# baggepinnen/LPVSpectral.jl

Measured on AMD Instinct MI355X. Metric: signals/sec, ls_sparse_spectral_lpv group lasso N=2^20 Nf=512 Nv=8 (2000 ADMM iters; iters/sec in admm_iters_per_sec), higher is better.
Workload: dtype f64

## Files before the change

lpvspectral.jl_amd/csrc/admm_pack.hip:

```cpp
#include "lpvs_internal.h"
#include "admm_device.h"
#include "admm_host.h"

#include <algorithm>
#include <map>
#include <mutex>
#include <tuple>
#include <vector>
#include <cmath>
#include <cstdlib>
#include <string>
#include <type_traits>

namespace lpvs {

namespace {

__global__ void __launch_bounds__(256)
pack_tiles_f32_kernel(const double *__restrict__ M, int64_t np, float *__restrict__ Mp) {
    int I, J;
    tile_index(blockIdx.x, I, J);
    const double2 *src = reinterpret_cast<const double2 *>(M + (int64_t)I * TS * np + (int64_t)J * TS);
    float2 *dst = reinterpret_cast<float2 *>(Mp + (int64_t)blockIdx.x * TS * TS);
    for (int e = threadIdx.x; e < TS * TS / 2; e += 256) {
// ... 27 lines not shown
}

__global__ void __launch_bounds__(256)
pack_tiles_split_kernel(const double *__restrict__ M, int64_t np, unsigned char *__restrict__ Mp) {
    int I, J;
    tile_index(blockIdx.x, I, J);
    M += (int64_t)blockIdx.y * np * np;
    Mp += (size_t)blockIdx.y * gridDim.x * kSplitTileBytes;
    const double *src = M + (int64_t)I * TS * np + (int64_t)J * TS;
    float *head = reinterpret_cast<float *>(Mp + (size_t)blockIdx.x * kSplitTileBytes);
    unsigned short *tail = reinterpret_cast<unsigned short *>(Mp + (size_t)blockIdx.x * kSplitTileBytes + (size_t)TS * TS * 4);
    for (int e = threadIdx.x; e < TS * TS; e += 256) {
        const int r = e >> 7, col = e & 127;
        const double m = src[(int64_t)r * np + col];
        unsigned long long B = (unsigned long long)__double_as_longlong(m);
        B = (B + (1ull << 12)) & ~((1ull << 13) - 1);
        float h = (float)__longlong_as_double((long long)(B & ~((1ull << 29) - 1)));
        unsigned int q = (unsigned int)(B >> 13) & 0xffffu;
        if (!(fabs(m) >= 0x1p-120) || !(fabs(m) < 0x1p127)) { h = (float)m; q = 0; }
        head[e] = h;
        tail[r * TS + 8 * ((col & 63) >> 2) + 4 * (col >> 6) + (col & 3)] = (unsigned short)q;
    }
}

__global__ void __launch_bounds__(256)
absmax_kernel(const double *__restrict__ M, int64_t np, int64_t n, unsigned long long *__restrict__ out) {
    M += (int64_t)blockIdx.y * np * np;
    out += blockIdx.y;
    double m = 0.0;
    for (int64_t i = (int64_t)blockIdx.x * 256 + threadIdx.x; i < n; i += (int64_t)gridDim.x * 256) m = fmax(m, fabs(M[i * np + i]));
#pragma unroll
    for (int w = 32; w >= 1; w >>= 1) m = fmax(m, __shfl_xor(m, w, 64));
    if ((threadIdx.x & 63) == 0 && m > 0.0) atomicMax(out, (unsigned long long)__double_as_longlong(m));
}

__global__ void __launch_bounds__(256)
pack_tiles_mixed_kernel(const double *__restrict__ M, int64_t np, unsigned char *__restrict__ Mp, unsigned char *__restrict__ types,
                        const unsigned long long *__restrict__ absmax_bits, double step_scale, int diag_float ,
                        double *__restrict__ abs1 , double *__restrict__ abs2 ,
                        int fix_drop_bits ) {
    int I, J;
    tile_index(blockIdx.x, I, J);
    M += (int64_t)blockIdx.y * np * np;
    Mp += (size_t)blockIdx.y * gridDim.x * kSplitTileBytes;
    types += (size_t)blockIdx.y * gridDim.x;
    absmax_bits += blockIdx.y;
    const double *src = M + (int64_t)I * TS * np + (int64_t)J * TS;
    unsigned char *slot = Mp + (size_t)blockIdx.x * kSplitTileBytes;
    __shared__ float rowstep[TS];
    __shared__ int bad;
    __shared__ double colabs[4][TS];
    const int lane = threadIdx.x & 63, wave = threadIdx.x >> 6;
    if (threadIdx.x == 0) bad = (diag_float && I == J) ? 1 : 0;
    __syncthreads();
    {
        const double limit = __longlong_as_double((long long)*absmax_bits) * step_scale;
        double c0 = 0.0, c1 = 0.0;
        for (int r = wave; r < TS; r += 4) {
            const double a0 = fabs(src[(int64_t)r * np + lane]), a1 = fabs(src[(int64_t)r * np + 64 + lane]);
            if (abs1 != nullptr) {
                c0 += a0; c1 += a1;
                const double rs = wave_sum(a0 + a1);
                if (lane == 0) abs1[(size_t)blockIdx.x * TS + r] = rs;
            }
            const double e0 = (I == J && lane == r) ? 0.0 : a0;
            const double e1 = (I == J && 64 + lane == r) ? 0.0 : a1;
            double m = fmax(e0, e1);
#pragma unroll
            for (int w = 32; w >= 1; w >>= 1) m = fmax(m, __shfl_xor(m, w, 64));
            if (lane == 0) {
                int e = 0;
                (void)frexp(m, &e);
                const double st = ldexp(1.0, e - 35);
                rowstep[r] = m > 0.0 ? (float)st : 0x1p-100f;
                if (m > 0.0 && (!(st <= limit) || e - 35 < -120)) atomicOr(&bad, 1);
            }
        }
        if (abs1 != nullptr) { colabs[wave][lane] = c0; colabs[wave][64 + lane] = c1; }
    }
    __syncthreads();
    if (abs2 != nullptr && threadIdx.x < TS)
        abs2[(size_t)blockIdx.x * TS + threadIdx.x] = ((colabs[0][threadIdx.x] + colabs[1][threadIdx.x]) + colabs[2][threadIdx.x]) + colabs[3][threadIdx.x];
    const bool fixed = !bad;
    if (threadIdx.x == 0) types[blockIdx.x] = fixed ? (I == J ? 2 : 1) : 0;
    if (!fixed) {
        float *head = reinterpret_cast<float *>(slot);
        unsigned short *tail = reinterpret_cast<unsigned short *>(slot + (size_t)TS * TS * 4);
        for (int e = threadIdx.x; e < TS * TS; e += 256) {
            const int r = e >> 7, col = e & 127;
            const double m = src[(int64_t)r * np + col];
            unsigned long long B = (unsigned long long)__double_as_longlong(m);
            B = (B + (1ull << 12)) & ~((1ull << 13) - 1);
            float h = (float)__longlong_as_double((long long)(B & ~((1ull << 29) - 1)));
            unsigned int q = (unsigned int)(B >> 13) & 0xffffu;
            if (!(fabs(m) >= 0x1p-120) || !(fabs(m) < 0x1p127)) { h = (float)m; q = 0; }
            head[e] = h;
            tail[r * TS + 8 * ((col & 63) >> 2) + 4 * (col >> 6) + (col & 3)] = (unsigned short)q;
        }
        return;
    }
    const double drop = (double)(1 << fix_drop_bits), drop_inv = 1.0 / drop;
    unsigned int *hi = reinterpret_cast<unsigned int *>(slot);
    unsigned int *nib = reinterpret_cast<unsigned int *>(slot + kFixHeadBytes);
    float *steps = reinterpret_cast<float *>(slot + kFixHeadBytes + kFixNibBytes);
    const int g = lane >> 4, c = lane & 15;
    for (int rg = 0; rg < 8; ++rg) {
        const int r = wave * 32 + 4 * rg + g;
        const double inv = 1.0 / (double)rowstep[r];
        unsigned int word = 0;
#pragma unroll
        for (int k = 0; k < 8; ++k) {
            const int col = k < 4 ? 4 * c + k : 64 + 4 * c + (k - 4);
            double qd = (I == J && col == r) ? 0.0 : rint(src[(int64_t)r * np + col] * inv * drop_inv) * drop;
            qd = fmin(fmax(qd, -0x1p35 + 1.0), 0x1p35 - 1.0);
            const unsigned long long q = (unsigned long long)((long long)qd + (1ll << 35));
            hi[r * TS + col] = (unsigned int)(q >> 4);
            word |= (unsigned int)(q & 15) << (4 * k);
        }
        nib[(wave * 64 + lane) * 8 + rg] = word;
        if (c == 0) steps[(wave * 4 + g) * 8 + rg] = rowstep[r];
    }
    if (I == J && threadIdx.x < TS)
        reinterpret_cast<double *>(slot + kFixHeadBytes + kFixNibBytes + TS * 4)[threadIdx.x] = src[(int64_t)threadIdx.x * np + threadIdx.x];
}

}

int32_t launch_pack_tiles_batch(const double *M, int64_t np, int nbatch, double *Mp, hipStream_t s) {
    const int nblk = (int)(np / TS);
    hipLaunchKernelGGL(pack_tiles_kernel, dim3((unsigned)(nblk * (nblk + 1) / 2), (unsigned)nbatch), dim3(256), 0, s, M, np, Mp);
    LPVS_HIP(hipGetLastError());
    return LPVS_OK;
}

size_t symv_part_doubles(int64_t np, int64_t ns) {
    const int64_t nblk = np / TS;
    return ((size_t)(nblk * (nblk + 1) / 2) * TS * 2 + 2 * (size_t)nblk + 2) * (size_t)ns + 16;
}
size_t symv_packed_doubles(int64_t np) {
    const int64_t nblk = np / TS;
    return (size_t)(nblk * (nblk + 1) / 2) * TS * TS;
}

int32_t launch_pack_tiles_f32(const double *M, int64_t np, float *Mp, hipStream_t s) {
    const int nblk = (int)(np / TS);
    hipLaunchKernelGGL(pack_tiles_f32_kernel, dim3((unsigned)(nblk * (nblk + 1) / 2)), dim3(256), 0, s, M, np, Mp);
    LPVS_HIP(hipGetLastError());
    return LPVS_OK;
}

int32_t launch_cvt_f32_f64(const float *src, double *dst, int64_t count, hipStream_t s) {
    if (count <= 0) return LPVS_OK;
    hipLaunchKernelGGL(cvt_f32_f64_kernel, dim3((unsigned)ceil_div(count, 256)), dim3(256), 0, s, src, dst, count);
// ... 67 lines not shown
```

lpvspectral.jl_amd/csrc/api.hip:

```cpp
#include <cmath>
#include <cstdarg>
#include <cstdio>
#include <cstdlib>
#include <cstring>
#include <ctime>
#include <map>
#include <mutex>
#include <array>
#include <thread>
#include <string>
#include <vector>

#include "lpvs_internal.h"

namespace lpvs {

static thread_local char g_err[512] = "";

void set_error(const char *fmt, ...) {
    va_list ap;
    va_start(ap, fmt);
    vsnprintf(g_err, sizeof(g_err), fmt, ap);
    va_end(ap);
}
// ... 448 lines not shown

AdmmParams make_params(const lpvs_problem *h) {
    const StoragePlan &pl = h->plan;
    const bool sym = h->np >= kSymmetricMinNp;
    AdmmParams p{h->M.as<double>(), h->np, h->n, h->bs.as<double>(), h->x.as<double>(), h->z.as<double>(), h->u.as<double>(),
                 h->rhs.as<double>(), h->mu, h->tol, h->prox_kind, h->prox_param, h->group_len, h->status.as<AdmmStatus>(),
                 h->scratch.as<double>(), h->part.as<double>(), sym ? h->Mp.as<double>() : nullptr, (int)h->ns};
    p.mp_f32 = pl.mode == kMpF32 ? 1 : 0;
    p.mp_split = pl.mode == kMpSplit || pl.mode == kMpMixed ? 1 : 0;
    p.mp_types = pl.mode == kMpMixed ? mp_tile_types(h->Mp, h->np, 1) : nullptr;
    p.mp_fix32 = p.mp_types != nullptr && (pl.fix_bits <= 32 || pl.nib_period > 0) ? 1 : 0;
    p.nib_period = pl.nib_period; p.nib_ramp = pl.nib_ramp; p.xb_corr = h->xb_corr.as<double>(); p.nib_rhs = h->nib_rhs.as<double>(); p.nib_part = h->nib_part.as<double>(); p.nib_acc = h->nib_acc.as<long long>();
    p.xb = pl.offset_form ? h->xb.as<double>() : nullptr;
    p.fi = pl.owns_fi && h->fi.p ? h->fi.as<double>() : nullptr;
    p.fi_R = h->fi_R; p.fi_xbmax = h->fi_xbmax;
    p.fi_prefetch_all = pl.mode == kMpMixed && h->Mp_census.fixed == h->Mp_census.total ? 1 : 0;
    p.opt_iteration = h->opt[LPVS_OPT_ITERATION]; p.opt_nt_loads = h->opt[LPVS_OPT_NT_LOADS];
    {
        const char *e = experiment_env("LPVS_TILE_ORDER");
        p.tile_order = p.fi != nullptr && !(e && std::string(e) == "forward") ? 1 : 0;
    }
    p.sm_ctl = !sym && h->sm_ctl.p ? h->sm_ctl.as<int>() : nullptr;
    p.prox_params = h->prox_per_signal && h->ns > 1 ? h->prox_params.as<double>() : nullptr;
    return p;
}

int32_t factorize(lpvs_problem *h, double shift) {
    if (h->M_valid && h->M_shift == shift) return LPVS_OK;
    const int64_t np = h->np, n = h->n;
    h->Mp_valid = false; h->Mp_rowsum = 0;
    if (!h->M.p) LPVS_TRY(h->M.alloc(sizeof(double) * (size_t)np * (size_t)np));
    if (!h->work.p) LPVS_TRY(h->work.alloc(spd_inverse_work_bytes(np)));
    LPVS_HIP(hipEventRecord(h->ev[3].a, h->stream));
    LPVS_HIP(hipMemcpyAsync(h->M.p, h->G.p, sizeof(double) * (size_t)np * (size_t)np, hipMemcpyDeviceToDevice, h->stream));
    LPVS_TRY(launch_add_diag(h->M.as<double>(), np, n, shift, h->stream));
    LPVS_TRY(spd_inverse_inplace(h->M.as<double>(), np, h->work.as<double>(), h->istat.as<int>(), h->stream, &h->res->aux));
    LPVS_HIP(hipEventRecord(h->ev[3].b, h->stream));
    int st = 0;
    LPVS_HIP(hipMemcpyAsync(&st, h->istat.p, sizeof(int), hipMemcpyDeviceToHost, h->stream));
    LPVS_HIP(hipStreamSynchronize(h->stream));
    h->t_factor += h->ev[3].ms();
    if (st != 0) {
        h->M_valid = false;
        set_error("(G + %.3g I) is not positive definite (non-positive pivot in the block sweep)", shift);
        return LPVS_ENUMERIC;
    }
    h->M_valid = true; h->M_shift = shift;
    return LPVS_OK;
}


StoragePlan decide_plan(lpvs_problem *h) {
    const int xc_opt = option_in_effect(LPVS_OPT_XUPDATE_CORRECTION, h->opt[LPVS_OPT_XUPDATE_CORRECTION]);
    const bool corrected = h->np >= kSymmetricMinNp && xc_opt != LPVS_XCORR_OFF;
    h->xcorr = xcorr_schedule_from(corrected ? experiment_env("LPVS_XUPDATE_CORRECTION") : nullptr, xcorr_default_schedule(h->ns, corrected));
    const int storage = option_in_effect(LPVS_OPT_M_STORAGE, h->opt[LPVS_OPT_M_STORAGE]);
    return admm_storage_plan(h->np, h->ns, h->f32, storage, h->ns > 1 && multi_signal_fixed_tiles_ok(h->np), h->xcorr.on(), fix_bits_from(experiment_env),
                             nib_knobs_from(experiment_env));
}

int32_t pack_mixed(lpvs_problem *h, const StoragePlan &want, StoragePlan *stored) {
    hipStream_t s = h->stream;
    const PackedLayout lay = packed_layout(h->np, want.element_bytes, 1);
    unsigned char *types = mp_tile_types(h->Mp, h->np, 1);
    unsigned long long *amax = reinterpret_cast<unsigned long long *>(h->Mp.as<unsigned char>() + lay.absmax_off);
    LPVS_TRY(launch_pack_tiles_mixed(h->M.as<double>(), h->np, h->Mp.as<unsigned char>(), types, amax, s, want.diag_float,
                                     want.want_rowsum ? h->part.as<double>() : nullptr, h->n, want.want_rowsum ? h->scratch.as<double>() : nullptr, want.fix_bits));
    std::vector<unsigned char> ht(lay.tiles);
// ... 2134 lines not shown
```

lpvspectral.jl_amd/csrc/linalg.hip:

```cpp
#include "lpvs_internal.h"
#include "factor_plan.h"

#include <cstdlib>
#include <map>
#include <mutex>
#include <string>
#include <vector>

namespace lpvs {

namespace {

typedef double f64x4 __attribute__((ext_vector_type(4)));
constexpr int NB = 64;

__global__ void __launch_bounds__(256)
diag_inverse_kernel(const double *__restrict__ Aall, int64_t np, int k, double *__restrict__ Pall, int *status,
                    int64_t strideA, int64_t strideW) {
    __shared__ double colp[NB], rowp[NB];
    const double *A = Aall + (int64_t)blockIdx.x * strideA;
    double *P = Pall + (int64_t)blockIdx.x * strideW;
    const double *blk = A + (int64_t)k * NB * np + (int64_t)k * NB;
    const int ti = threadIdx.x >> 4, tj = threadIdx.x & 15;
    double v[4][4];
// ... 864 lines not shown
            }
        }
        __syncthreads();
    }
    if (skip_wave) return;
    if (below) {
#pragma unroll
        for (int i = 0; i < 2; ++i)
#pragma unroll
            for (int r = 0; r < 4; ++r) {
                double *sp = A + (r_lo + i * 16 + 4 * r) * np + c_lo;
#pragma unroll
                for (int j = 0; j < 2; ++j) *reinterpret_cast<double *>(reinterpret_cast<char *>(sp + j * 16) + voffb) = acc[i][j][r];
            }
        return;
    }
#pragma unroll
    for (int i = 0; i < 2; ++i)
#pragma unroll
        for (int j = 0; j < 2; ++j)
#pragma unroll
            for (int r = 0; r < 4; ++r) {
                const int64_t row = r_lo + i * 16 + lk + 4 * r, col = c_lo + j * 16 + li;
                if (col <= row) A[row * np + col] = acc[i][j][r];
            }
}

__global__ void __launch_bounds__(256) add_diag_kernel(double *__restrict__ Mall, int64_t np, int64_t n, double shift) {
    const int64_t i = (int64_t)blockIdx.x * 256 + threadIdx.x;
    double *M = Mall + (int64_t)blockIdx.y * np * np;
    if (i < np) M[i * np + i] = i < n ? M[i * np + i] + shift : 1.0;
}

__global__ void __launch_bounds__(256) negate_mirror_kernel(double *__restrict__ Aall, int64_t np) {
    __shared__ double tile[32][33];
    double *A = Aall + (int64_t)blockIdx.z * np * np;
    const int bi = blockIdx.y, bj = blockIdx.x;
    if (bj > bi) return;
    const int tx = threadIdx.x & 31, ty = threadIdx.x >> 5;
    const int64_t r0 = (int64_t)bi * 32, c0 = (int64_t)bj * 32;
    for (int r = ty; r < 32; r += 8) {
        const double v = -A[(r0 + r) * np + c0 + tx];
        tile[r][tx] = v;
        if (bi != bj || tx <= r) A[(r0 + r) * np + c0 + tx] = v;
    }
    __syncthreads();
    for (int r = ty; r < 32; r += 8)
        if (bi != bj || tx > r) A[(c0 + r) * np + r0 + tx] = tile[tx][r];
}

__global__ void __launch_bounds__(256)
symm_matmul_kernel(const double *__restrict__ A, const double *__restrict__ B, double *__restrict__ C, int64_t np) {
    const int lane = threadIdx.x & 63, wave = threadIdx.x >> 6;
    const int64_t r0 = ((int64_t)blockIdx.y * 2 + (wave >> 1)) * 64, c0 = ((int64_t)blockIdx.x * 2 + (wave & 1)) * 64;
    const int li = lane & 15, lk = lane >> 4;
    f64x4 acc[4][4];
#pragma unroll
    for (int i = 0; i < 4; ++i)
#pragma unroll
        for (int j = 0; j < 4; ++j) acc[i][j] = (f64x4){0.0, 0.0, 0.0, 0.0};
    for (int64_t kk = 0; kk < np; kk += 4) {
        double opA[4], opB[4];
#pragma unroll
        for (int q = 0; q < 4; ++q) {
            opA[q] = A[(kk + lk) * np + r0 + q * 16 + li];
            opB[q] = B[(kk + lk) * np + c0 + q * 16 + li];
// ... 325 lines not shown
    }
    return factor_steps_serial(c, plan);
}

static int32_t spd_inverse_impl(double *A, int64_t np, int nbatch, double *work, int *status_dev, hipStream_t s, SweepAux *aux) {
    if (np % 128 != 0) { set_error("spd_inverse: np=%lld not a multiple of 128", (long long)np); return LPVS_ESTATE; }
    LPVS_HIP(hipMemsetAsync(status_dev, 0, sizeof(int) * (size_t)nbatch, s));
    const FactorPlan plan = factor_plan(np, nbatch, aux != nullptr, factor_knobs_from(experiment_env));
    if (plan.level == FactorLevel::two) {
        LPVS_TRY(spd_inverse_two_level(A, np, work, status_dev, s, aux, plan));
    } else {
        sweep64(A, np, nbatch, work, status_dev, s);
        LPVS_HIP(hipGetLastError());
    }
    hipLaunchKernelGGL(negate_mirror_kernel, dim3((unsigned)(np / 32), (unsigned)(np / 32), (unsigned)nbatch), dim3(256), 0, s, A, np);
    LPVS_HIP(hipGetLastError());
    return LPVS_OK;
}

int32_t spd_inverse_inplace_batch(double *A, int64_t np, int nbatch, double *work, int *status_dev, hipStream_t s) {
    return spd_inverse_impl(A, np, nbatch, work, status_dev, s, nullptr);
}

int32_t spd_inverse_inplace(double *A, int64_t np, double *work, int *status_dev, hipStream_t s, SweepAux *aux) {
    return spd_inverse_impl(A, np, 1, work, status_dev, s, aux);
}

int32_t launch_add_diag_batch(double *M, int64_t np, int64_t n, double shift, int nbatch, hipStream_t s) {
    hipLaunchKernelGGL(add_diag_kernel, dim3((unsigned)ceil_div(np, 256), (unsigned)nbatch), dim3(256), 0, s, M, np, n, shift);
    LPVS_HIP(hipGetLastError());
    return LPVS_OK;
}

int32_t launch_add_diag(double *M, int64_t np, int64_t n, double shift, hipStream_t s) {
    hipLaunchKernelGGL(add_diag_kernel, dim3((unsigned)ceil_div(np, 256)), dim3(256), 0, s, M, np, n, shift);
    LPVS_HIP(hipGetLastError());
    return LPVS_OK;
}

int32_t launch_symm_matmul(const double *A, const double *B, double *C, int64_t np, hipStream_t s) {
    if (np % 128 != 0) return LPVS_ESTATE;
    hipLaunchKernelGGL(symm_matmul_kernel, dim3((unsigned)(np / 128), (unsigned)(np / 128)), dim3(256), 0, s, A, B, C, np);
    LPVS_HIP(hipGetLastError());
    return LPVS_OK;
}

}
```

lpvspectral.jl_amd/csrc/lpvs_internal.h:

```cpp
#pragma once
#include <hip/hip_runtime.h>
#include <exception>
#include <new>
#include <stdint.h>
#include <functional>
#include <string>
#include <vector>

#include "../../include/lpvspectral.h"
#include "windows_plan.h"
#include "admm_plan.h"
#include "gram_form_plan.h"
#include "eval_plan.h"

namespace lpvs {

inline const char *experiment_env(const char *name) {
#ifdef LPVS_NO_EXPERIMENTS
    (void)name;
    return nullptr;
#else
    const char *on = getenv("LPVS_EXPERIMENTS");
    return (on && on[0] == '1') ? getenv(name) : nullptr;
#endif
// ... 137 lines not shown
int32_t launch_nufft_window_modes(const double *grids, int64_t grid_bstride, int nwin, int nf, int mode0, int nslots, const double *scale_dev, double *tab,
                                  int64_t tab_bstride, hipStream_t s);
int32_t launch_ap_assemble_fourier(const double *tab, const double *eps, int64_t Nf, int64_t s0, double delta, int zf, int64_t n, double *G,
                                   int64_t ldg, int nbatch, int64_t tab_stride, int64_t g_stride, hipStream_t s);
int32_t launch_ap_rhs_fourier(const double *tab, const double *eps, int64_t Nf, int zf, double *b, int nbatch, int64_t tab_stride,
                              int64_t b_stride, hipStream_t s);
int32_t launch_ap_assemble(const double *tab, const double *eps, int64_t Nf, int64_t s0, double delta, int64_t nb, int64_t n, double *G,
                           int64_t ldg, hipStream_t s);
int32_t launch_ap_rhs(const double *tab, const double *eps, int64_t Nf, int64_t nb, double *b, hipStream_t s);

struct EvalBasis {
    const double *vc = nullptr;
    int nb = 1;
    double gamma = 0;
    int normalize = 0, coulomb = 0;
};
int32_t launch_eval_direct(const double *x, const double *v, const double *y, int64_t M, const double *w_dev, int64_t Nf, const double *P_dev, int64_t nc,
                           const EvalBasis &B, double scale, double *out, double *part, hipStream_t s);
int32_t launch_eval_grids(const double *Q_dev, int64_t ngrids, int64_t Nf, int nf, double *tw_dev, double *grids_dev, hipStream_t s);
int32_t launch_eval_interp(const double *x, const double *v, const double *y, int64_t M, double a, double D_hi, double D_lo, int nf, const double *grids_dev,
                           bool twin, int64_t nc, const EvalBasis &B, double scale, double *out, double *part, hipStream_t s);
int32_t launch_eval_sums(const double *part, int64_t M, int64_t nc, double *sums_dev, hipStream_t s);

struct SweepAux {
    hipStream_t side = nullptr;
    hipStream_t bulk = nullptr;
    hipEvent_t panel = nullptr, rest = nullptr, band = nullptr, second = nullptr, bulkdone = nullptr;
    int32_t ensure();
    ~SweepAux();
};
size_t spd_inverse_work_bytes(int64_t np);
int32_t spd_inverse_inplace(double *A, int64_t np, double *work, int *status_dev, hipStream_t s, SweepAux *aux = nullptr);
int32_t launch_add_diag(double *M, int64_t np, int64_t n, double shift, hipStream_t s);
int32_t launch_add_diag_batch(double *M, int64_t np, int64_t n, double shift, int nbatch, hipStream_t s);
int32_t spd_inverse_inplace_batch(double *A, int64_t np, int nbatch, double *work, int *status_dev, hipStream_t s);
int32_t launch_symm_matmul(const double *A, const double *B, double *C, int64_t np, hipStream_t s);

struct AdmmStatus {
    long long iters;
    int converged;
    int pad;
    double nxz;
};
struct AdmmParams {
    const double *M;
    int64_t np;
    int64_t n;
    const double *b;
    double *x, *z, *u, *rhs;
    double mu, tol;
    int prox_kind;
    double prox_param;
    int64_t group_len;
    AdmmStatus *status;
    double *scratch;
    double *part;
    const double *Mp;
    int ns;
    int mp_f32 = 0;
    int mp_split = 0;
    int nib_period = 0;
    int nib_ramp = 0;
    int mp_fix32 = 0;
    const double *xb_corr = nullptr;
    double *nib_rhs = nullptr;
    long long *nib_acc = nullptr;
// ... 124 lines not shown
```

lpvspectral.jl_amd/csrc/nufft.hip:

```cpp
#include "lpvs_internal.h"
#include "nufft_bins.h"
#include "nufft_coord.h"

#include <cmath>
#include <cstring>
#include <map>
#include <mutex>
#include <vector>

namespace lpvs {
namespace {

constexpr int NU_W = kNuWidth;
static int nu_gpw(int nf) { return nu_scatter_gpw(nf); }
constexpr double NU_MAGIC = 6755399441055744.0;
constexpr int NU_CHUNK = kNuChunk;

__global__ void __launch_bounds__(256)
nufft_coord_kernel(const double *__restrict__ x, int64_t N, double D_hi, double D_lo, int nf, int *__restrict__ cell0, double *__restrict__ taps) {
    const int64_t i = (int64_t)blockIdx.x * 256 + threadIdx.x;
    if (i >= N) return;
    int g0;
    const double p = nu_grid_pos(nu_phase_turns(D_hi, D_lo, x[i]), nf, &g0);
    cell0[i] = (g0 + nf) & (nf - 1);
// ... 194 lines not shown
    const int gamma = blockIdx.x, q = gamma >> 1, twin = gamma & 1;
    const int ntw = HALF ? nf >> 1 : nf;
    for (int g = threadIdx.x; g < nf; g += 256) {
        Gd[g] = grid[(int64_t)gamma * nf + g];
        if (g < ntw) {
            double sn, cs;
            sincospi(2.0 * (double)g / (double)nf, &sn, &cs);
            tw[g] = make_double2(cs, sn);
        }
    }
    __syncthreads();
    const int j = blockIdx.y * 256 + threadIdx.x;
    if (j >= nslots) return;
    double ac0 = 0, as0 = 0, ac1 = 0, as1 = 0;
    int idx = 0;
    const int mask = nf - 1, mj = (mode0 + j) & mask;
    const int hmask = mask >> 1, hbit = nf >> 1;
    for (int g = 0; g < nf; g += 2) {
        const double2 t0 = tw[HALF ? idx & hmask : idx];
        const bool n0 = HALF && (idx & hbit);
        idx = (idx + mj) & mask;
        const double2 t1 = tw[HALF ? idx & hmask : idx];
        const bool n1 = HALF && (idx & hbit);
        idx = (idx + mj) & mask;
        double v0 = Gd[g], v1 = Gd[g + 1];
        if (HALF) { v0 = n0 ? -v0 : v0; v1 = n1 ? -v1 : v1; }
        ac0 = fma(v0, t0.x, ac0); as0 = fma(v0, t0.y, as0);
        ac1 = fma(v1, t1.x, ac1); as1 = fma(v1, t1.y, as1);
    }
    const double sc = scale[(int64_t)gamma * scale_stride + j];
    double *o = tab + ((int64_t)j * nq + q) * 4 + 2 * twin;
    o[0] = (ac0 + ac1) * sc;
    o[1] = (as0 + as1) * sc;
}


__global__ void __launch_bounds__(256)
nufft_window_kernel(const double *__restrict__ x, const double *__restrict__ W, const double *__restrict__ yA, const double *__restrict__ yB, int hasB,
                    const int64_t *__restrict__ offs, int64_t n, double D_hi, double D_lo, int nf, double *__restrict__ gridA,
                    double *__restrict__ gridB, int64_t grid_bstride) {
    extern __shared__ __attribute__((aligned(16))) long long G[];
    __shared__ unsigned long long smax[4];
    const int win = blockIdx.x;
    const int64_t r0 = offs[win];
    const int ng = hasB ? 4 : 2;
    for (int e = threadIdx.x; e < ng * nf; e += 256) G[e] = 0;
    if (threadIdx.x < 4) smax[threadIdx.x] = 0;
    __syncthreads();
    {
        double m[4] = {0, 0, 0, 0};
        for (int64_t i = threadIdx.x; i < n; i += 256) {
            const double xv = fabs(x[r0 + i]), wv = W ? W[i] : 1.0;
            const double cA = fabs(yA ? wv * yA[r0 + i] : wv), cB = hasB ? fabs(wv * yB[r0 + i]) : 0.0;
            m[0] = fmax(m[0], cA); m[1] = fmax(m[1], xv * cA); m[2] = fmax(m[2], cB); m[3] = fmax(m[3], xv * cB);
            if (!(xv * cA < 1.0 / 0.0)) m[0] = m[1] = 1.0 / 0.0;
            if (!(xv * cB < 1.0 / 0.0)) m[2] = m[3] = 1.0 / 0.0;
        }
#pragma unroll
        for (int g = 0; g < 4; ++g)
            if (m[g] > 0.0) atomicMax(&smax[g], (unsigned long long)__double_as_longlong(m[g]));
    }
    __syncthreads();
    double quantum[4], iq[4];
#pragma unroll
    for (int g = 0; g < 4; ++g) {
        const double bound = __longlong_as_double((long long)smax[g]) * (double)n;
// ... 111 lines not shown
        for (int twin = 0; twin < 2; ++twin) {
            const double bound = (twin ? xam : 1.0) * cmax * (double)N;
            int e = 0;
            (void)std::frexp(bound > 0 ? bound : 1.0, &e);
            const double quantum = std::ldexp(1.0, e - 62);
            hquantum[(size_t)(2 * q + twin)] = quantum;
            hinvq[(size_t)(2 * q + twin)] = bound > 0 ? 1.0 / quantum : 0.0;
        }
    }
    LPVS_TRY(copy_to_device(invq, hinvq.data(), sizeof(double) * hinvq.size(), s));
    const size_t lds_spread = sizeof(long long) * (size_t)gpw * (size_t)nf;
    if (!scatter) {
        const NuGatherPlan plan = nu_gather_plan(N, nf, nq);
        hipLaunchKernelGGL(nufft_gather_kernel, dim3((unsigned)plan.nblocks), dim3(256), 0, s, x, y, Wt, ldw, nq, N, nf, cell0, taps, perm, bin_start, invq,
                           partial, plan);
    } else if (gpw == 4) {
        LPVS_HIP(hipFuncSetAttribute(reinterpret_cast<const void *>(&nufft_spread_kernel<4>), hipFuncAttributeMaxDynamicSharedMemorySize, (int)lds_spread));
        hipLaunchKernelGGL(nufft_spread_kernel<4>, dim3((unsigned)(8 * ngroups * ceil_div(nchunks, 8))), dim3(256), lds_spread, s, x, y, Wt, ldw, nq, N, nf, cell0,
                           taps, invq, partial, ngroups, nchunks);
    } else {
        LPVS_HIP(hipFuncSetAttribute(reinterpret_cast<const void *>(&nufft_spread_kernel<2>), hipFuncAttributeMaxDynamicSharedMemorySize, (int)lds_spread));
        hipLaunchKernelGGL(nufft_spread_kernel<2>, dim3((unsigned)(8 * ngroups * ceil_div(nchunks, 8))), dim3(256), lds_spread, s, x, y, Wt, ldw, nq, N, nf, cell0,
                           taps, invq, partial, ngroups, nchunks);
    }
    hipLaunchKernelGGL(nufft_reduce_kernel, dim3((unsigned)ceil_div(nf, 256), (unsigned)(2 * nq)), dim3(256), 0, s, partial, ngroups, nchunks, nf, gpw, grid);
    LPVS_HIP(hipGetLastError());
    {
        std::vector<double> hscale((size_t)(2 * nq) * (size_t)nslots);
        const std::vector<long double> phat = nufft_phihat(nf, mode0 + nslots);
        for (int g = 0; g < 2 * nq; ++g)
            for (int j = 0; j < nslots; ++j) hscale[(size_t)g * (size_t)nslots + (size_t)j] = (double)((long double)hquantum[(size_t)g] / phat[(size_t)(mode0 + j)]);
        LPVS_TRY(copy_to_device(scale, hscale.data(), sizeof(double) * hscale.size(), s));
    }
    if (nf <= 4096) {
        const size_t lds_modes = sizeof(double) * 3 * (size_t)nf;
        LPVS_HIP(hipFuncSetAttribute(reinterpret_cast<const void *>(&nufft_modes_kernel<false>), hipFuncAttributeMaxDynamicSharedMemorySize, (int)lds_modes));
        hipLaunchKernelGGL(nufft_modes_kernel<false>, dim3((unsigned)(2 * nq), (unsigned)ceil_div(nslots, 256)), dim3(256), lds_modes, s, grid, nf, nq, mode0,
                           nslots, scale, tab, (int64_t)nslots, (int64_t)0, (int64_t)0);
    } else {
        const size_t lds_modes = sizeof(double) * 2 * (size_t)nf;
        LPVS_HIP(hipFuncSetAttribute(reinterpret_cast<const void *>(&nufft_modes_kernel<true>), hipFuncAttributeMaxDynamicSharedMemorySize, (int)lds_modes));
        hipLaunchKernelGGL(nufft_modes_kernel<true>, dim3((unsigned)(2 * nq), (unsigned)ceil_div(nslots, 256)), dim3(256), lds_modes, s, grid, nf, nq, mode0,
                           nslots, scale, tab, (int64_t)nslots, (int64_t)0, (int64_t)0);
    }
    LPVS_HIP(hipGetLastError());
    return LPVS_OK;
}


std::vector<double> nufft_window_scale(int nf, int mode0, int nslots) {
    const std::vector<long double> phat = nufft_phihat(nf, mode0 + nslots);
    std::vector<double> r((size_t)nslots);
    for (int j = 0; j < nslots; ++j) r[(size_t)j] = (double)(1.0L / phat[(size_t)(mode0 + j)]);
    return r;
}
int32_t launch_nufft_window_spread(const double *x, const double *W, const double *yA, const double *yB, bool hasB, const int64_t *offs_dev, int nwin,
                                   int64_t n, double D_hi, double D_lo, int nf, double *gridA, double *gridB, int64_t grid_bstride, hipStream_t s) {
    const size_t lds = sizeof(long long) * 4 * (size_t)nf;
    LPVS_HIP(hipFuncSetAttribute(reinterpret_cast<const void *>(&nufft_window_kernel), hipFuncAttributeMaxDynamicSharedMemorySize, (int)lds));
    hipLaunchKernelGGL(nufft_window_kernel, dim3((unsigned)nwin), dim3(256), lds, s, x, W, yA, yB, hasB ? 1 : 0, offs_dev, n, D_hi, D_lo, nf, gridA, gridB,
                       grid_bstride);
    LPVS_HIP(hipGetLastError());
    return LPVS_OK;
}
int32_t launch_nufft_window_modes(const double *grids, int64_t grid_bstride, int nwin, int nf, int mode0, int nslots, const double *scale_dev, double *tab,
                                  int64_t tab_bstride, hipStream_t s) {
    const size_t lds_modes = sizeof(double) * 3 * (size_t)nf;
// ... 9 lines not shown
```

Before: 15.40.

## Batch pack-kernel row reductions, fuse shifted copy, and tile NUFFT mode evaluation

The mixed-tile pack kernel now loads 16 rows per wave at once and reduces them with a butterfly shuffle that leaves one row result per lane group. Its fixed-point encoding pass gains coalesced row loads and a shuffle-based nibble assembly. The separate device copy plus add-diagonal before the SPD inverse becomes one kernel that copies only the lower-triangle tiles and applies the shift. A new tiled NUFFT modes kernel, on by default, processes 8 grids per block with double-buffered LDS and a twiddle table, replacing the per-grid kernel. The lower-only copy assumes the inverse reads only the lower triangle of M.

```diff
diff --git a/lpvspectral.jl_amd/csrc/admm_pack.hip b/lpvspectral.jl_amd/csrc/admm_pack.hip
--- a/lpvspectral.jl_amd/csrc/admm_pack.hip
+++ b/lpvspectral.jl_amd/csrc/admm_pack.hip
@@ -83,6 +83,31 @@
 #pragma unroll
     for (int w = 32; w >= 1; w >>= 1) m = fmax(m, __shfl_xor(m, w, 64));
     if ((threadIdx.x & 63) == 0 && m > 0.0) atomicMax(out, (unsigned long long)__double_as_longlong(m));
+}
+
+constexpr int kPackRows = 16;
+__device__ __forceinline__ int rows16_owner_row(int lane) { return ((lane >> 5) & 1) | ((lane >> 3) & 2) | ((lane >> 1) & 4) | ((lane << 1) & 8); }
+template <class Term, class Op>
+__device__ __forceinline__ double rows16_reduce(Term term, int lane, Op op) {
+    double x[kPackRows / 2];
+    const bool up0 = (lane & 32) != 0;
+#pragma unroll
+    for (int j = 0; j < kPackRows / 2; ++j) {
+        const double a = term(2 * j), b = term(2 * j + 1);
+        x[j] = op(up0 ? b : a, __shfl_xor(up0 ? a : b, 32, 64));
+    }
+#pragma unroll
+    for (int k = 1; k < 4; ++k) {
+        const bool up = (lane & (32 >> k)) != 0;
+#pragma unroll
+        for (int j = 0; j < kPackRows / 4; ++j)
+            if (j < (kPackRows / 2 >> k)) {
+                const double keep = up ? x[2 * j + 1] : x[2 * j], send = up ? x[2 * j] : x[2 * j + 1];
+                x[j] = op(keep, __shfl_xor(send, 32 >> k, 64));
+            }
+    }
+    x[0] = op(x[0], __shfl_xor(x[0], 2, 64));
+    return op(x[0], __shfl_xor(x[0], 1, 64));
 }
 
 __global__ void __launch_bounds__(256)
@@ -107,23 +132,32 @@
     {
         const double limit = __longlong_as_double((long long)*absmax_bits) * step_scale;
         double c0 = 0.0, c1 = 0.0;
-        for (int r = wave; r < TS; r += 4) {
-            const double a0 = fabs(src[(int64_t)r * np + lane]), a1 = fabs(src[(int64_t)r * np + 64 + lane]);
+#pragma unroll 1
+        for (int i0 = 0; i0 < TS / 4; i0 += kPackRows) {
+            double a0[kPackRows], a1[kPackRows];
+#pragma unroll
+            for (int i = 0; i < kPackRows; ++i) {
+                a0[i] = fabs(src[(int64_t)(wave + 4 * (i0 + i)) * np + lane]);
+                a1[i] = fabs(src[(int64_t)(wave + 4 * (i0 + i)) * np + 64 + lane]);
+            }
+            const int rown = wave + 4 * (i0 + rows16_owner_row(lane));
             if (abs1 != nullptr) {
-                c0 += a0; c1 += a1;
-                const double rs = wave_sum(a0 + a1);
-                if (lane == 0) abs1[(size_t)blockIdx.x * TS + r] = rs;
+#pragma unroll
+                for (int i = 0; i < kPackRows; ++i) { c0 += a0[i]; c1 += a1[i]; }
+                const double rs = rows16_reduce([&](int i) { return a0[i] + a1[i]; }, lane, [](double a, double b) { return a + b; });
+                if ((lane & 3) == 0) abs1[(size_t)blockIdx.x * TS + rown] = rs;
             }
-            const double e0 = (I == J && lane == r) ? 0.0 : a0;
-            const double e1 = (I == J && 64 + lane == r) ? 0.0 : a1;
-            double m = fmax(e0, e1);
-#pragma unroll
-            for (int w = 32; w >= 1; w >>= 1) m = fmax(m, __shfl_xor(m, w, 64));
-            if (lane == 0) {
+            const double m = rows16_reduce([&](int i) {
+                const int r = wave + 4 * (i0 + i);
+                const double e0 = (I == J && lane == r) ? 0.0 : a0[i];
+                const double e1 = (I == J && 64 + lane == r) ? 0.0 : a1[i];
+                return fmax(e0, e1);
+            }, lane, [](double a, double b) { return fmax(a, b); });
+            if ((lane & 3) == 0) {
                 int e = 0;
                 (void)frexp(m, &e);
                 const double st = ldexp(1.0, e - 35);
-                rowstep[r] = m > 0.0 ? (float)st : 0x1p-100f;
+                rowstep[rown] = m > 0.0 ? (float)st : 0x1p-100f;
                 if (m > 0.0 && (!(st <= limit) || e - 35 < -120)) atomicOr(&bad, 1);
             }
         }
@@ -154,22 +188,32 @@
     unsigned int *hi = reinterpret_cast<unsigned int *>(slot);
     unsigned int *nib = reinterpret_cast<unsigned int *>(slot + kFixHeadBytes);
     float *steps = reinterpret_cast<float *>(slot + kFixHeadBytes + kFixNibBytes);
-    const int g = lane >> 4, c = lane & 15;
-    for (int rg = 0; rg < 8; ++rg) {
-        const int r = wave * 32 + 4 * rg + g;
-        const double inv = 1.0 / (double)rowstep[r];
-        unsigned int word = 0;
-#pragma unroll
-        for (int k = 0; k < 8; ++k) {
-            const int col = k < 4 ? 4 * c + k : 64 + 4 * c + (k - 4);
-            double qd = (I == J && col == r) ? 0.0 : rint(src[(int64_t)r * np + col] * inv * drop_inv) * drop;
-            qd = fmin(fmax(qd, -0x1p35 + 1.0), 0x1p35 - 1.0);
-            const unsigned long long q = (unsigned long long)((long long)qd + (1ll << 35));
-            hi[r * TS + col] = (unsigned int)(q >> 4);
-            word |= (unsigned int)(q & 15) << (4 * k);
+    auto fix = [&](int r, int col, double m, double inv) {
+        double qd = (I == J && col == r) ? 0.0 : rint(m * inv * drop_inv) * drop;
+        qd = fmin(fmax(qd, -0x1p35 + 1.0), 0x1p35 - 1.0);
+        return (unsigned long long)__double_as_longlong(qd + (0x1p52 + 0x1p35)) & ((1ull << 52) - 1);
+    };
+#pragma unroll 1
+    for (int i0 = 0; i0 < TS / 4; i0 += 8) {
+        double v0[8], v1[8];
+#pragma unroll
+        for (int i = 0; i < 8; ++i) {
+            v0[i] = src[(int64_t)(wave + 4 * (i0 + i)) * np + lane];
+            v1[i] = src[(int64_t)(wave + 4 * (i0 + i)) * np + 64 + lane];
         }
-        nib[(wave * 64 + lane) * 8 + rg] = word;
-        if (c == 0) steps[(wave * 4 + g) * 8 + rg] = rowstep[r];
+#pragma unroll
+        for (int i = 0; i < 8; ++i) {
+            const int r = wave + 4 * (i0 + i);
+            const double inv = 1.0 / (double)rowstep[r];
+            const unsigned long long q0 = fix(r, lane, v0[i], inv), q1 = fix(r, 64 + lane, v1[i], inv);
+            hi[r * TS + lane] = (unsigned int)(q0 >> 4);
+            hi[r * TS + 64 + lane] = (unsigned int)(q1 >> 4);
+            unsigned int word = ((unsigned int)(q0 & 15) << (4 * (lane & 3))) | ((unsigned int)(q1 & 15) << (4 * (4 + (lane & 3))));
+            word |= (unsigned int)__shfl_xor((int)word, 1, 64);
+            word |= (unsigned int)__shfl_xor((int)word, 2, 64);
+            if ((lane & 3) == 0) nib[((r >> 5) * 64 + (r & 3) * 16 + (lane >> 2)) * 8 + ((r & 31) >> 2)] = word;
+            if (lane == 0) steps[((r >> 5) * 4 + (r & 3)) * 8 + ((r & 31) >> 2)] = rowstep[r];
+        }
     }
     if (I == J && threadIdx.x < TS)
         reinterpret_cast<double *>(slot + kFixHeadBytes + kFixNibBytes + TS * 4)[threadIdx.x] = src[(int64_t)threadIdx.x * np + threadIdx.x];
diff --git a/lpvspectral.jl_amd/csrc/api.hip b/lpvspectral.jl_amd/csrc/api.hip
--- a/lpvspectral.jl_amd/csrc/api.hip
+++ b/lpvspectral.jl_amd/csrc/api.hip
@@ -504,8 +504,7 @@
     if (!h->M.p) LPVS_TRY(h->M.alloc(sizeof(double) * (size_t)np * (size_t)np));
     if (!h->work.p) LPVS_TRY(h->work.alloc(spd_inverse_work_bytes(np)));
     LPVS_HIP(hipEventRecord(h->ev[3].a, h->stream));
-    LPVS_HIP(hipMemcpyAsync(h->M.p, h->G.p, sizeof(double) * (size_t)np * (size_t)np, hipMemcpyDeviceToDevice, h->stream));
-    LPVS_TRY(launch_add_diag(h->M.as<double>(), np, n, shift, h->stream));
+    LPVS_TRY(launch_shifted_copy_lower(h->G.as<double>(), h->M.as<double>(), np, n, shift, h->stream));
     LPVS_TRY(spd_inverse_inplace(h->M.as<double>(), np, h->work.as<double>(), h->istat.as<int>(), h->stream, &h->res->aux));
     LPVS_HIP(hipEventRecord(h->ev[3].b, h->stream));
     int st = 0;
diff --git a/lpvspectral.jl_amd/csrc/linalg.hip b/lpvspectral.jl_amd/csrc/linalg.hip
--- a/lpvspectral.jl_amd/csrc/linalg.hip
+++ b/lpvspectral.jl_amd/csrc/linalg.hip
@@ -920,6 +920,26 @@
     if (i < np) M[i * np + i] = i < n ? M[i * np + i] + shift : 1.0;
 }
 
+__global__ void __launch_bounds__(256)
+shifted_copy_lower_kernel(const double *__restrict__ G, double *__restrict__ M, int64_t np, int64_t n, double shift) {
+    const int tr = blockIdx.y, tc = blockIdx.x;
+    if (tc > tr && !(tc == tr + 1 && (tr & 1) == 0)) return;
+    const int lane = threadIdx.x & 63, wave = threadIdx.x >> 6;
+    const int64_t c = (int64_t)tc * 128 + 2 * lane;
+    for (int r0 = wave; r0 < 128; r0 += 32) {
+        double2 v[8];
+#pragma unroll
+        for (int k = 0; k < 8; ++k) v[k] = *reinterpret_cast<const double2 *>(G + ((int64_t)tr * 128 + r0 + 4 * k) * np + c);
+#pragma unroll
+        for (int k = 0; k < 8; ++k) {
+            const int64_t i = (int64_t)tr * 128 + r0 + 4 * k;
+            if (i == c) v[k].x = i < n ? v[k].x + shift : 1.0;
+            if (i == c + 1) v[k].y = i < n ? v[k].y + shift : 1.0;
+            *reinterpret_cast<double2 *>(M + i * np + c) = v[k];
+        }
+    }
+}
+
 __global__ void __launch_bounds__(256) negate_mirror_kernel(double *__restrict__ Aall, int64_t np) {
     __shared__ double tile[32][33];
     double *A = Aall + (int64_t)blockIdx.z * np * np;
@@ -1311,6 +1331,13 @@
     return LPVS_OK;
 }
 
+int32_t launch_shifted_copy_lower(const double *G, double *M, int64_t np, int64_t n, double shift, hipStream_t s) {
+    if (np % 128 != 0) { set_error("spd_inverse: np=%lld not a multiple of 128", (long long)np); return LPVS_ESTATE; }
+    hipLaunchKernelGGL(shifted_copy_lower_kernel, dim3((unsigned)(np / 128), (unsigned)(np / 128)), dim3(256), 0, s, G, M, np, n, shift);
+    LPVS_HIP(hipGetLastError());
+    return LPVS_OK;
+}
+
 int32_t launch_add_diag(double *M, int64_t np, int64_t n, double shift, hipStream_t s) {
     hipLaunchKernelGGL(add_diag_kernel, dim3((unsigned)ceil_div(np, 256)), dim3(256), 0, s, M, np, n, shift);
     LPVS_HIP(hipGetLastError());
diff --git a/lpvspectral.jl_amd/csrc/lpvs_internal.h b/lpvspectral.jl_amd/csrc/lpvs_internal.h
--- a/lpvspectral.jl_amd/csrc/lpvs_internal.h
+++ b/lpvspectral.jl_amd/csrc/lpvs_internal.h
@@ -193,6 +193,7 @@
 size_t spd_inverse_work_bytes(int64_t np);
 int32_t spd_inverse_inplace(double *A, int64_t np, double *work, int *status_dev, hipStream_t s, SweepAux *aux = nullptr);
 int32_t launch_add_diag(double *M, int64_t np, int64_t n, double shift, hipStream_t s);
+int32_t launch_shifted_copy_lower(const double *G, double *M, int64_t np, int64_t n, double shift, hipStream_t s);
 int32_t launch_add_diag_batch(double *M, int64_t np, int64_t n, double shift, int nbatch, hipStream_t s);
 int32_t spd_inverse_inplace_batch(double *A, int64_t np, int nbatch, double *work, int *status_dev, hipStream_t s);
 int32_t launch_symm_matmul(const double *A, const double *B, double *C, int64_t np, hipStream_t s);
diff --git a/lpvspectral.jl_amd/csrc/nufft.hip b/lpvspectral.jl_amd/csrc/nufft.hip
--- a/lpvspectral.jl_amd/csrc/nufft.hip
+++ b/lpvspectral.jl_amd/csrc/nufft.hip
@@ -250,6 +250,116 @@
     double *o = tab + ((int64_t)j * nq + q) * 4 + 2 * twin;
     o[0] = (ac0 + ac1) * sc;
     o[1] = (as0 + as1) * sc;
+}
+
+constexpr int kModesTile = 8, kModesChunk = 128, kModesStep = 8;
+template <bool HALF, int MJ>
+__global__ void __launch_bounds__(256)
+nufft_modes_tiled_kernel(const double *__restrict__ grid, int nf, int nq, int mode0, int nslots, const double *__restrict__ scale ,
+                         double *__restrict__ tab) {
+    extern __shared__ __attribute__((aligned(16))) double lds[];
+    const int ntw = HALF ? nf >> 1 : nf;
+    double2 *tw = reinterpret_cast<double2 *>(lds);
+    double *buf = lds + 2 * ntw;
+    const int t = threadIdx.x, gl = t & (kModesTile - 1), jl = t >> 3;
+    const int gamma0 = blockIdx.x * kModesTile, ngam = 2 * nq;
+    const int scell = t & (kModesChunk - 1), sg0 = t >> 7;
+    double st[4];
+#pragma unroll
+    for (int k = 0; k < 4; ++k) {
+        const int ga = gamma0 + sg0 + 2 * k;
+        st[k] = ga < ngam ? grid[(int64_t)ga * nf + scell] : 0.0;
+    }
+    for (int g = t; g < ntw; g += 256) {
+        double sn, cs;
+        sincospi(2.0 * (double)g / (double)nf, &sn, &cs);
+        tw[g] = make_double2(cs, sn);
+    }
+#pragma unroll
+    for (int k = 0; k < 4; ++k) buf[scell * kModesTile + sg0 + 2 * k] = st[k];
+    __syncthreads();
+    const int mask = nf - 1, hmask = mask >> 1, hbit = nf >> 1;
+    const int jb = blockIdx.y * (32 * MJ) + jl;
+    int mj[MJ], idx[MJ];
+    double ac0[MJ], as0[MJ], ac1[MJ], as1[MJ];
+#pragma unroll
+    for (int m = 0; m < MJ; ++m) {
+        mj[m] = (mode0 + jb + 32 * m) & mask;
+        idx[m] = 0;
+        ac0[m] = as0[m] = ac1[m] = as1[m] = 0;
+    }
+    const int nchunks = nf / kModesChunk;
+    for (int c = 0; c < nchunks; ++c) {
+        if (c + 1 < nchunks) {
+#pragma unroll
+            for (int k = 0; k < 4; ++k) {
+                const int ga = gamma0 + sg0 + 2 * k;
+                st[k] = ga < ngam ? grid[(int64_t)ga * nf + (c + 1) * kModesChunk + scell] : 0.0;
+            }
+        }
+        const double *B = buf + (c & 1) * (kModesChunk * kModesTile) + gl;
+        double wA[kModesStep], wB[kModesStep];
+        double2 tA[MJ][kModesStep], tB[MJ][kModesStep];
+        unsigned nA[MJ], nB[MJ];
+        auto fetch = [&](const double *Bg, double (&w)[kModesStep], double2 (&t)[MJ][kModesStep], unsigned (&neg)[MJ]) {
+#pragma unroll
+            for (int u = 0; u < kModesStep; ++u) w[u] = Bg[u * kModesTile];
+#pragma unroll
+            for (int m = 0; m < MJ; ++m) {
+                neg[m] = 0;
+#pragma unroll
+                for (int u = 0; u < kModesStep; ++u) {
+                    t[m][u] = tw[HALF ? idx[m] & hmask : idx[m]];
+                    if (HALF && (idx[m] & hbit)) neg[m] |= 1u << u;
+                    idx[m] = (idx[m] + mj[m]) & mask;
+                }
+            }
+        };
+        auto sum = [&](const double (&w)[kModesStep], const double2 (&t)[MJ][kModesStep], const unsigned (&neg)[MJ]) {
+#pragma unroll
+            for (int m = 0; m < MJ; ++m)
+#pragma unroll
+                for (int u = 0; u < kModesStep; u += 2) {
+                    double v0 = w[u], v1 = w[u + 1];
+                    if (HALF) { v0 = (neg[m] >> u) & 1u ? -v0 : v0; v1 = (neg[m] >> (u + 1)) & 1u ? -v1 : v1; }
+                    ac0[m] = fma(v0, t[m][u].x, ac0[m]); as0[m] = fma(v0, t[m][u].y, as0[m]);
+                    ac1[m] = fma(v1, t[m][u + 1].x, ac1[m]); as1[m] = fma(v1, t[m][u + 1].y, as1[m]);
+                }
+        };
+        fetch(B, wA, tA, nA);
+#pragma unroll 1
+        for (int g = 0; g < kModesChunk - 2 * kModesStep; g += 2 * kModesStep) {
+            fetch(B + (g + kModesStep) * kModesTile, wB, tB, nB);
+            __builtin_amdgcn_sched_barrier(0);
+            sum(wA, tA, nA);
+            __builtin_amdgcn_sched_barrier(0);
+            fetch(B + (g + 2 * kModesStep) * kModesTile, wA, tA, nA);
+            __builtin_amdgcn_sched_barrier(0);
+            sum(wB, tB, nB);
+            __builtin_amdgcn_sched_barrier(0);
+        }
+        fetch(B + (kModesChunk - kModesStep) * kModesTile, wB, tB, nB);
+        __builtin_amdgcn_sched_barrier(0);
+        sum(wA, tA, nA);
+        sum(wB, tB, nB);
+        if (c + 1 < nchunks) {
+            double *Wn = buf + ((c + 1) & 1) * (kModesChunk * kModesTile);
+#pragma unroll
+            for (int k = 0; k < 4; ++k) Wn[scell * kModesTile + sg0 + 2 * k] = st[k];
+        }
+        __syncthreads();
+    }
+    const int gamma = gamma0 + gl, q = gamma >> 1, twin = gamma & 1;
+    if (gamma >= ngam) return;
+#pragma unroll
+    for (int m = 0; m < MJ; ++m) {
+        const int j = jb + 32 * m;
+        if (j >= nslots) continue;
+        const double sc = scale[(int64_t)gamma * nslots + j];
+        double *o = tab + ((int64_t)j * nq + q) * 4 + 2 * twin;
+        o[0] = (ac0[m] + ac1[m]) * sc;
+        o[1] = (as0[m] + as1[m]) * sc;
+    }
 }
 
 
@@ -427,7 +537,19 @@
             for (int j = 0; j < nslots; ++j) hscale[(size_t)g * (size_t)nslots + (size_t)j] = (double)((long double)hquantum[(size_t)g] / phat[(size_t)(mode0 + j)]);
         LPVS_TRY(copy_to_device(scale, hscale.data(), sizeof(double) * hscale.size(), s));
     }
-    if (nf <= 4096) {
+    const char *modes_knob = experiment_env("LPVS_NUFFT_MODES");
+    const bool per_grid = modes_knob && strcmp(modes_knob, "per-grid") == 0;
+    if (!per_grid) {
+        const bool half = nf > 4096;
+        const size_t lds_modes = sizeof(double) * (size_t)(half ? nf : 2 * nf) + sizeof(double) * 2 * kModesChunk * kModesTile;
+        const unsigned gtiles = (unsigned)ceil_div(2 * nq, kModesTile);
+        const bool two = modes_knob && strcmp(modes_knob, "one") == 0 ? false : modes_knob && strcmp(modes_knob, "two") == 0 ? true
+                         : (int64_t)gtiles * ceil_div(nslots, 64) >= 128;
+        auto *kern = half ? (two ? &nufft_modes_tiled_kernel<true, 2> : &nufft_modes_tiled_kernel<true, 1>)
+                          : (two ? &nufft_modes_tiled_kernel<false, 2> : &nufft_modes_tiled_kernel<false, 1>);
+        LPVS_HIP(hipFuncSetAttribute(reinterpret_cast<const void *>(kern), hipFuncAttributeMaxDynamicSharedMemorySize, (int)lds_modes));
+        hipLaunchKernelGGL(kern, dim3(gtiles, (unsigned)ceil_div(nslots, two ? 64 : 32)), dim3(256), lds_modes, s, grid, nf, nq, mode0, nslots, scale, tab);
+    } else if (nf <= 4096) {
         const size_t lds_modes = sizeof(double) * 3 * (size_t)nf;
         LPVS_HIP(hipFuncSetAttribute(reinterpret_cast<const void *>(&nufft_modes_kernel<false>), hipFuncAttributeMaxDynamicSharedMemorySize, (int)lds_modes));
         hipLaunchKernelGGL(nufft_modes_kernel<false>, dim3((unsigned)(2 * nq), (unsigned)ceil_div(nslots, 256)), dim3(256), lds_modes, s, grid, nf, nq, mode0,
```

Result: no change. 15.50 (median of 6 runs) (+0.6%).
